# amberxie88/latent_diffusion_planning

Measured on AMD Instinct MI355X. Metric: latent plans/sec (horizon=9, 100 DDIM steps), higher is better.
Workload: dtype f32; 1 GPU; configs[1]: rm_lift planner ConditionalUnet1D (D=25, T=8, down_dims [256,512,1024]), 100-step DDIM, batch 256 synthetic latents per GPU, random-init weights, Philox noise, hipGraph-captured loop; plans_per_gpu=256, denoise_steps=100, sampler=ddim, graph=True, parallelism=dp1, ranks_seen_by_backend=1, backend=none, range_fallback=0, fp16_plane_launches=0

## Files before the change

### latent_diffusion_planning_amd/csrc/engine.hip

```cpp
#include "engine.hpp"
#include "sconv.hpp"
#include "t2pack.hpp"
#include "t4pack.hpp"
#include "version.h"

#include <algorithm>
#include <cmath>
#include <cstring>

namespace ldp {

void betas_squaredcos(int n, std::vector<float>& betas, std::vector<float>& alphas,
                             std::vector<float>& acp) {
  auto abar = [](double t) {
    const double c = std::cos((t + 0.008) / 1.008 * M_PI / 2.0);
    return c * c;
  };
  betas.resize(n);
  alphas.resize(n);
  acp.resize(n);
  float run = 1.0f;
  for (int i = 0; i < n; ++i) {
    const double b = std::min(1.0 - abar((double)(i + 1) / n) / abar((double)i / n), 0.999);
    betas[i] = (float)b;
    alphas[i] = 1.0f - betas[i];
    run = run * alphas[i];
    acp[i] = run;
  }
}

void make_step_coefs(int n_train, int n_steps, int sampler, std::vector<StepCoef>& out) {
  std::vector<float> betas, alphas, acp;
  betas_squaredcos(n_train, betas, alphas, acp);
  out.assign(n_steps, StepCoef{});
  const int stride = n_train / n_steps;
  for (int i = 0; i < n_steps; ++i) {
// ... 187 lines not shown
  const HostTensor& t = it->second;
  if (t.shape.size() != shape.size() || !std::equal(shape.begin(), shape.end(), t.shape.begin())) {
    std::string got, want;
    for (auto s : t.shape) got += std::to_string(s) + ",";
    for (auto s : shape) want += std::to_string(s) + ",";
    return fail(LDP_EINVAL, "weight '%s' has shape (%s) expected (%s)", path.c_str(), got.c_str(),
                want.c_str());
  }
  *out = &t;
  return LDP_OK;
}

static int upload_padded(DevBuf& dst, const float* src, int n, int n_p, float fill, hipStream_t s) {
  std::vector<float> tmp(n_p, fill);
  std::copy(src, src + n, tmp.begin());
  LDP_TRY(dst.alloc((size_t)n_p * 4));
  LDP_HIP(hipMemcpy(dst.p, tmp.data(), (size_t)n_p * 4, hipMemcpyHostToDevice));
  (void)s;
  return LDP_OK;
}

int make_conv(ldp_handle* h, const std::string& prefix, int nj, int cin, int cout, int cin_p,
              int cout_p, const char* gn_prefix, hipStream_t s, ConvW& out, int t_pos) {
  const HostTensor *k = nullptr, *b = nullptr;
  LDP_TRY(get_weight(h, prefix + "/kernel", &k, {nj, cin, cout}));
  LDP_TRY(get_weight(h, prefix + "/bias", &b, {cout}));
  out.t2s = nj == 5 && t2_shared(MODE_K5, t_pos, 0);
  out.t4s = nj == 5 && t4_shared(MODE_K5, t_pos, 0);
  std::vector<float> packed = out.t2s ? pack_conv_t2(k->data.data(), nullptr, cin, cout, cin_p, cout_p)
                            : out.t4s ? pack_conv_t4(k->data.data(), nullptr, cin, cout, cin_p, cout_p)
                                      : pack_conv(k->data.data(), nj, cin, cout, cin_p, cout_p);
  LDP_TRY(out.w.alloc(packed.size() * 4));
  LDP_HIP(hipMemcpy(out.w.p, packed.data(), packed.size() * 4, hipMemcpyHostToDevice));
  LDP_TRY(upload_padded(out.bias, b->data.data(), cout, cout_p, 0.f, s));
  out.nj = nj; out.cin = cin; out.cout = cout; out.cin_p = cin_p; out.cout_p = cout_p;
  out.has_gn = gn_prefix != nullptr;
  out.wsplit.release(); out.wsplit16.release(); out.wsplit16h.release(); out.wsplith.release();
  out.f16_refused = false;
  if (gn_prefix) {
    const HostTensor *gs = nullptr, *gb = nullptr;
    LDP_TRY(get_weight(h, std::string(gn_prefix) + "/scale", &gs, {cout}));
    LDP_TRY(get_weight(h, std::string(gn_prefix) + "/bias", &gb, {cout}));
    LDP_TRY(upload_padded(out.gn_scale, gs->data.data(), cout, cout_p, 1.f, s));
    LDP_TRY(upload_padded(out.gn_bias, gb->data.data(), cout, cout_p, 0.f, s));
  }
  return LDP_OK;
}

static int add_res_proj(ldp_handle* h, const std::string& conv_prefix, const std::string& prefix, int cin,
                        int cout, int cin_p, ConvW& c) {
  const HostTensor *k = nullptr, *b = nullptr, *kc = nullptr;
  LDP_TRY(get_weight(h, prefix + "/kernel", &k, {1, cin, cout}));
  LDP_TRY(get_weight(h, prefix + "/bias", &b, {cout}));
  LDP_TRY(get_weight(h, conv_prefix + "/kernel", &kc, {c.nj, cin, cout}));
  c.wsplit.release(); c.wsplit16.release(); c.wsplit16h.release(); c.wsplith.release();
  c.f16_refused = false;
  std::vector<float> packed;
  if (c.t2s) {
    packed = pack_conv_t2(kc->data.data(), k->data.data(), cin, cout, cin_p, c.cout_p);
  } else if (c.t4s) {
    packed = pack_conv_t4(kc->data.data(), k->data.data(), cin, cout, cin_p, c.cout_p);
  } else {
    std::vector<float> both(kc->data);
    both.insert(both.end(), k->data.begin(), k->data.end());
    packed = pack_conv(both.data(), c.nj + 1, cin, cout, cin_p, c.cout_p);
  }
  LDP_TRY(c.w.alloc(packed.size() * 4));
  LDP_HIP(hipMemcpy(c.w.p, packed.data(), packed.size() * 4, hipMemcpyHostToDevice));
  LDP_TRY(c.bres.alloc((size_t)cout * 4));
  LDP_HIP(hipMemcpy(c.bres.p, b->data.data(), (size_t)cout * 4, hipMemcpyHostToDevice));
  c.has_res = true;
  return LDP_OK;
}

static int round_up(int v, int m) { return (v + m - 1) / m * m; }

static int pick_plan(int mode, int to, int cout, int cin_total, int ca, bool res_out, ConvPlan& p,
                     int* cs_io = nullptr, int mb_want = 1, bool up_full_depth = false) {
  const int gw = cout >= 256 ? cout / 8 : 32;
  if (cs_io && *cs_io == 4) {
    const int qb = gw / 4;
    int ks4 = 0, cpi4 = 0;
    if (mode == MODE_K5) {
      if (to == 2 && qb == 32) { ks4 = 4; cpi4 = 2; }
      else if (to == 4 && qb == 16) { ks4 = 8; cpi4 = 1; }
      else if (to == 8 && qb == 16) { ks4 = 8; cpi4 = 1; }
      else if (to == 4 && qb == 32) { ks4 = 4; cpi4 = res_out ? 1 : 2; }
    }
    const int chunk4 = 16 * ks4 * cpi4;
// ... 63 lines not shown
    else if (to == 4 && bn == 128) { ks = 1; cpi = 2; }
    else if (to == 4 && bn == 32) { if (cin_total % 128 == 0) { ks = 4; cpi = 2; } else { ks = 2; cpi = 1; } }
    else if (to == 2 && bn == 32) { ks = 4; cpi = 1; }
  }
  if (ks == 0)
    return fail(LDP_EINVAL, "no MFMA conv instantiation for mode=%d T_out=%d C_out=%d (group width %d)",
                mode, to, cout, bn);
  p = ConvPlan{mode, to, nwn, ks, cpi, res_out ? 1 : 0};
  if (mb_want == 2 && mode == MODE_K5 &&
      ((to == 4 && !res_out && (bn == 64 || bn == 32)) || (to == 2 && (bn == 128 || bn == 64))))
    p.mb = 2;
  if (cin_total % p.chunk() != 0 || ca % p.chunk() != 0)
    return fail(LDP_EINVAL, "input channels (%d, first part %d) not a multiple of the %d-channel chunk "
                "(mode=%d T_out=%d C_out=%d)", cin_total, ca, p.chunk(), mode, to, cout);
  return LDP_OK;
}

static int launch_conv(ldp_handle* h, const ConvPlan& p, const ConvArgs& a_in, hipStream_t s) {
  const int dbg = h->opt.dbg, repeat = h->opt.repeat;
  ConvArgs a = a_in;
  a.dbg = dbg;
  if (h->opt.timeline_ptr && h->last_conv_launches < 64)
    a.tl = reinterpret_cast<unsigned long long*>(h->opt.timeline_ptr) + (size_t)h->last_conv_launches * 131072;
  if (!(a.flags & EP_STEP))
    for (int i = 1; i < repeat; ++i) (void)tconv_launch(p, a, s);
  const int r = tconv_launch(p, a, s);
  h->plan_log[plan_key(p)]++;
  h->last_conv_launches++;
  h->last_total_launches++;
  if (p.mb == 2 && p.to == 4 && (p.split == 2 || p.split == 3)) h->stat_mb2_launches++;
  if (p.split >= 3) h->stat_f16_launches++;
  if (t2_shared(p.mode, p.to, p.split)) h->stat_t2_shared_launches++;
  if (t4_shared(p.mode, p.to, p.split)) h->stat_t4_shared_launches++;
  if (r == -100)
    return fail(LDP_EINVAL, "conv instantiation missing: mode=%d TO=%d NWN=%d KS=%d CPI=%d res=%d",
                p.mode, p.to, p.nwn, p.ks, p.cpi, p.res_out);
  if (r != 0) return fail(LDP_EHIP, "conv launch failed: %s", hipGetErrorString((hipError_t)r));
  return LDP_OK;
}

static int block_positions(const PlannerState& P, size_t i) {
  const int nd = 2 * P.L;
  const int lvl = (int)i < nd ? (int)i / 2 : (int)i < nd + 2 ? P.L - 1 : P.L - 1 - ((int)i - nd - 2) / 2;
  return P.T >> lvl;
}

int planner_finalize(ldp_handle* h, hipStream_t s) {
  const ldp_config& c = h->cfg;
  PlannerState& P = h->pl;
  P = PlannerState{};
  P.D = c.obs_dim; P.DP = round_up(c.obs_dim, 32); P.G = c.global_cond_dim; P.T = c.pred_horizon;
  P.L = c.n_levels; P.E = c.step_embed_dim; P.n_train = c.planner_train_steps;
  P.C0P = P.DP <= 32 ? 128 : round_up(P.DP, 64);
  if (c.kernel_size != 5 || c.n_groups != 8)
    return fail(LDP_EINVAL, "only kernel_size=5 / n_groups=8 kernels are built (got %d / %d)",
                c.kernel_size, c.n_groups);
  if (P.L < 2 || P.L > LDP_MAX_LEVELS) return fail(LDP_EINVAL, "n_levels must be 2..%d", LDP_MAX_LEVELS);
  if (P.T % (1 << (P.L - 1)) != 0)
    return fail(LDP_EINVAL, "pred_horizon=%d is not a multiple of %d: the reference U-Net's skip "
                "connections cannot be concatenated (SURVEY.md fact 5)", P.T, 1 << (P.L - 1));
  P.dims.assign(c.down_dims, c.down_dims + P.L);
  for (int l = 0; l < P.L; ++l)
    if (P.dims[l] < 256 || P.dims[l] % 128 != 0)
      return fail(LDP_EINVAL, "down_dims[%d] = %d: every level must be >= 256 and a multiple of 128 "
                  "(8 GroupNorm groups of whole 16-column MFMA blocks)", l, P.dims[l]);
  const std::string root = "planner/";
// ... 383 lines not shown
    } else if (tile == 17) {
      p = ConvPlan{mode, to, p.bn() / 16, p.bn() == 32 ? 2 : 1, 2, 0};
      p.mb = 1; p.split = 1;
      a.w = w.wsplit16.f();
      if (h->f16_planner() && w.wsplit16h.p) { p.split = 3; a.w = w.wsplit16h.f(); }
      if (p.split == 3 && h->opt.planner_split_8w && ((B + 15) / 16) * 8 <= h->n_cu && ca % (32 * 2 * p.ks) == 0 &&
          ((mode == MODE_DOWN && ((to == 2 && p.nwn == 4) || (to == 4 && p.nwn == 2))) || (mode == MODE_UP && ((to == 4 && p.nwn == 4) || (to == 8 && p.nwn == 2)))))
        p.ks *= 2;
    } else if (tile == 16) {
      const int ks16 = p.bn() == 32 ? 2 : 1;
      const int cpi16 = 2;
      p = ConvPlan{MODE_K5, to, p.bn() / 16, ks16, cpi16, res_out ? 1 : 0};
      p.mb = 1; p.split = 1;
      a.w = w.wsplit16.f();
      if (h->opt.planner_split_mb2 && cs == 1 && to == 4 && p.bn() == 128 && ((B + 31) / 32) * 8 >= h->n_cu) {
        p = ConvPlan{MODE_K5, to, p.bn() / 16, 1, 2, res_out ? 1 : 0};
        p.mb = 2; p.split = 2;
      }
      if (h->f16_planner() && w.wsplit16h.p && res_out && to == 4 && p.bn() == 64 && p.cpi == 2 && p.ks == 1 && (ca + cb) % 64 == 0 && ca % 64 == 0) p.ks = 2;
      if (h->f16_planner() && w.wsplit16h.p && p.cpi == 2 && ((p.ks == 1 && (p.bn() == 128 || p.bn() == 64)) || (p.ks == 2 && (p.bn() == 32 || (p.bn() == 64 && res_out && to == 4)))) &&
          (to == 4 || to == 8 || (to == 16 && p.bn() == 32)) && !(to == 8 && p.bn() == 128)) {
        if (p.mb == 2 && res_out) p.mb = 1;
        p.split = 3;
        a.w = w.wsplit16h.f();
        if (h->opt.planner_split_8w && p.mb == 1 && p.nwn * p.ks == 4 && ((B + 15) / 16) * 8 <= h->n_cu && (ca + cb) % (32 * 2 * p.ks) == 0 && ca % (32 * 2 * p.ks) == 0 &&
            ((to == 8 && p.nwn == 2 && !res_out) || (to == 4 && p.nwn == 2) || (to == 4 && p.nwn == 4 && !res_out)))
          p.ks *= 2;
      }
    }
    if (p.split == 0 && mode == MODE_K5 && w.t2s != t2_shared(mode, to, 0))
      return fail(LDP_EINVAL, "k = 5 conv packed %s the shared-product form launched at %d positions", w.t2s ? "for" : "without", to);
    if (p.split == 0 && mode == MODE_K5 && w.t4s != t4_shared(mode, to, 0))
      return fail(LDP_EINVAL, "k = 5 conv packed %s the nine-product form launched at %d positions", w.t4s ? "for" : "without", to);
    a.bres = w.bres.f(); a.res_out = res_out;
    a.gn_scale = w.gn_scale.f(); a.gn_bias = w.gn_bias.f();
    if (film) {
      a.film_t = P.film_t.f() + film->film_off;
      a.film_g = P.film_g.f() + film->film_off;
      a.film_stride = P.F;
    }
    a.k_dev = k_dev; a.k = k;
    a.res_in = res_in; a.out = out;
    a.B = B; a.cout = w.cout_p; a.flags = flags; a.rows_valid = B * to;
    {
      const double wbytes = 4.0 * w.nj * (ca + cb) * w.cout_p, abytes = 4.0 * B * mode_ti(mode, to) * (ca + cb);
      const int thr = h->opt.by_sample;
      if (thr > 0 && a.kw <= 1 && (B + 15) / 16 <= 32768 && wbytes < (double)thr * abytes) a.by_sample = 1;
      else if (h->opt.place2d && p.split && a.kw <= 1) a.by_sample = 2;
    }
    if (!tap) return launch_conv(h, p, a, s);
    LDP_TRY(launch_conv(h, p, a, s));
    return tapped(p, a, tile, mode, to, w, xa, ca_stored, xb, cb, film);
  }

  int block(const ResBlock& b, int t, const float* xa, int ca, const float* xb, int cb, float* tmp,
            float* rbuf, float* out) {
    LDP_TRY(conv(b.c1, MODE_K5, t, xa, ca, xb, cb, tmp, EP_GN | EP_FILM, &b, nullptr,
                 b.proj ? rbuf : nullptr));
    const float* res = b.proj ? rbuf : xa;
    LDP_TRY(conv(b.c2, MODE_K5, t, tmp, b.cout, nullptr, 0, out, EP_GN | EP_RESIN, nullptr, res, nullptr));
    return LDP_OK;
  }
};
}

int planner_forward_launch(ldp_handle* h, int B, const int* k_dev, int k, bool step,
// ... 881 lines not shown
    if (v != 2) for (const auto& kv : h->plan_log) text[plan_text(kv.first)] = kv.second;
    for (const auto& kv : text) fprintf(stderr, "PLAN %s launches=%lld\n", kv.first.c_str(), (long long)kv.second);
    return LDP_OK;
  }
  else if (n == "inject_fault") { if (v && h->fault_host) h->fault_host[v == 2 ? 1 : 0] = 1u; return LDP_OK; }
  else return fail(LDP_EKEY, "unknown option '%s'", name);
  drop_graphs(h);
  return LDP_OK;
}

int ldp_get_option(ldp_handle* h, const char* name, int64_t* value) {
  if (!h || !name || !value) return fail(LDP_EINVAL, "bad argument");
  const std::string n(name);
  const Options& o = h->opt;
  if (n == "no_csplit") *value = o.no_csplit;
  else if (n == "no_mb2") *value = o.no_mb2;
  else if (n == "no_kw") *value = o.no_kw;
  else if (n == "kw_min_it") *value = o.kw_min_it;
  else if (n == "kw_bmax") *value = o.kw_bmax;
  else if (n == "no_fin_rows") *value = o.no_fin_rows;
  else if (n == "no_batch_split") *value = o.no_batch_split;
  else if (n == "up_full_depth") *value = o.up_full_depth;
  else if (n == "planner_split") *value = o.planner_split;
  else if (n == "planner_split_updown") *value = o.planner_split_updown;
  else if (n == "planner_split_cs2") *value = o.planner_split_cs2;
  else if (n == "planner_split_c256") *value = o.planner_split_c256;
  else if (n == "planner_split_mb2") *value = o.planner_split_mb2;
  else if (n == "planner_split_t2res") *value = o.planner_split_t2res;
  else if (n == "planner_split_t16") *value = o.planner_split_t16;
  else if (n == "planner_split_f16") *value = o.planner_split_f16;
  else if (n == "stat_f16_launches") *value = h->stat_f16_launches;
  else if (n == "stat_t2_shared_launches") *value = h->stat_t2_shared_launches;
  else if (n == "stat_t4_shared_launches") *value = h->stat_t4_shared_launches;
  else if (n == "stat_mb2_launches") *value = h->stat_mb2_launches;
  else if (n.rfind("stat_train_gemm_", 0) == 0) {
    static const char* const forms[3] = {"nn", "nt", "tn"};
    static const char* const tiles[5] = {"32", "32_ki2", "64", "64_ki2", "128"};
    const std::string rest = n.substr(16);
    int idx = rest == "fused" ? LDP_STAT_GEMM_FUSED : rest == "reduce" ? LDP_STAT_GEMM_REDUCE : -1;
    for (int f = 0; f < 3 && idx < 0; ++f)
      for (int t = 0; t < 5; ++t)
        if (rest == std::string(forms[f]) + "_" + tiles[t]) idx = f * 5 + t;
    if (idx < 0) return fail(LDP_EKEY, "unknown option '%s'", name);
    *value = h->stat_train_gemm[idx];
  }
  else if (n.rfind("stat_idm_", 0) == 0) {
    const std::string rest = n.substr(9);
    int idx = rest == "unfused" ? LDP_STAT_IDM_UNFUSED : rest == "f16_hs2" ? LDP_STAT_IDM_F16_HS2 : rest == "f16_hs4" ? LDP_STAT_IDM_F16_HS4 : -1;
    for (int hs = 1; hs <= 8 && idx < 0; hs *= 2)
      for (int ring = 0; ring <= (hs >= 4 ? 1 : 0); ++ring)
        for (int nt = 0; nt < 2; ++nt)
          if (rest == "f32_hs" + std::to_string(hs) + (ring ? "_ring" : "") + (nt ? "_nt" : "")) idx = stat_idm_f32(hs, ring != 0, nt != 0);
    if (idx < 0) return fail(LDP_EKEY, "unknown option '%s'", name);
    *value = h->stat_idm[idx];
  }
  else if (n == "vae_no_conv_stats") *value = o.vae_no_conv_stats;
  else if (n == "vae_no_conv_in_stats") *value = o.vae_no_conv_in_stats;
  else if (n == "vae_split") *value = o.vae_split;
  else if (n == "vae_split_f16") *value = o.vae_split_f16;
  else if (n == "vae_split_gn_only") *value = o.vae_split_gn_only;
  else if (n == "vae_split_s2") *value = o.vae_split_s2;
  else if (n == "timeline_ptr") *value = o.timeline_ptr;
  else if (n == "idm_unfused") *value = o.idm_unfused;
  else if (n == "idm_rt_major") *value = o.idm_rt_major;
  else if (n == "idm_noring") *value = o.idm_noring;
  else if (n == "idm_stream") *value = o.idm_stream;
// ... 37 lines not shown
                   int64_t n, void* stream) {
  if (!out_dev || n <= 0) return fail(LDP_EINVAL, "bad argument");
  return philox_raw_launch(seed, elem0, step, stream_id, out_dev, n, (hipStream_t)stream);
}

int ldp_philox_normal(uint64_t seed, uint64_t elem0, uint32_t step, uint32_t stream_id, float* out_dev,
                      int64_t n, void* stream) {
  if (!out_dev || n <= 0) return fail(LDP_EINVAL, "bad argument");
  return philox_normal_launch(seed, elem0, step, stream_id, out_dev, n, (hipStream_t)stream);
}

int ldp_launch_count(ldp_handle* h, int32_t which, int64_t* launches) {
  if (!h || !launches) return fail(LDP_EINVAL, "bad argument");
  *launches = which == 0 ? h->last_conv_launches : h->last_total_launches;
  return LDP_OK;
}

static int prim_conv(int mode, const float* x, const float* kernel_host, const float* bias_host,
                     const float* gs, const float* gb, const float* film, float* y, int B, int t_in,
                     int cin, int cout, void* stream) {
  if (!x || !kernel_host || !bias_host || !y || B <= 0) return fail(LDP_EINVAL, "bad argument");
  hipStream_t s = (hipStream_t)stream;
  const int nj = mode_taps(mode);
  const int to = mode == MODE_DOWN ? t_in / 2 : mode == MODE_UP ? t_in * 2 : t_in;
  if (cout % 128 != 0) return fail(LDP_EINVAL, "Cout must be a multiple of 128 (8 groups x 16)");
  ConvPlan p;
  int cin_pp = round_up(cin, 32);
  for (int pad = 64; pick_plan(mode, to, cout, cin_pp, cin_pp, false, p) != LDP_OK; pad *= 2) {
    if (pad > 256) return LDP_EINVAL;
    cin_pp = round_up(cin, pad);
  }
  std::vector<float> packed = t2_shared(mode, to, 0) ? pack_conv_t2(kernel_host, nullptr, cin, cout, cin_pp, cout)
                            : t4_shared(mode, to, 0) ? pack_conv_t4(kernel_host, nullptr, cin, cout, cin_pp, cout)
                                                     : pack_conv(kernel_host, nj, cin, cout, cin_pp, cout);
  DevBuf dw, db, dgs, dgb, dx, dfg, dft;
  LDP_TRY(upload(dw, packed.data(), packed.size() * 4, s));
  LDP_TRY(upload(db, bias_host, (size_t)cout * 4, s));
  ConvArgs a{};
  if (gs) {
    LDP_TRY(upload(dgs, gs, (size_t)cout * 4, s));
    LDP_TRY(upload(dgb, gb, (size_t)cout * 4, s));
    a.flags |= EP_GN;
  }
  const float* xin = x;
  if (cin_pp != cin) {
    LDP_TRY(dx.alloc((size_t)B * t_in * cin_pp * 4));
    LDP_TRY(pad_rows_launch(x, dx.f(), (int64_t)B * t_in, cin, cin_pp, s));
    xin = dx.f();
  }
  if (film) {
    LDP_TRY(dft.alloc((size_t)2 * cout * 4));
    LDP_HIP(hipMemsetAsync(dft.p, 0, (size_t)2 * cout * 4, s));
    a.film_t = dft.f(); a.film_g = film; a.film_stride = 2 * cout; a.flags |= EP_FILM;
  }
  a.xa = xin; a.ca = cin_pp; a.w = dw.f(); a.bias = db.f();
  a.gn_scale = dgs.f(); a.gn_bias = dgb.f();
  a.out = y; a.B = B; a.cout = cout; a.k = 0; a.rows_valid = B * to;
  const int r = tconv_launch(p, a, s);
  if (r != 0) return fail(r == -100 ? LDP_EINVAL : LDP_EHIP, "primitive conv launch failed (%d)", r);
  LDP_HIP(hipStreamSynchronize(s));
  return LDP_OK;
}

int ldp_conv1d_gn_mish_film_f32(const float* x, const float* kernel_host, const float* bias_host,
                                const float* gn_scale_host, const float* gn_bias_host,
                                const float* film, float* y, int32_t B, int32_t T, int32_t Cin,
// ... 19 lines not shown
```

### latent_diffusion_planning_amd/csrc/engine.hpp

```cpp
#pragma once
#include <functional>
#include <map>
#include <memory>
#include <string>
#include <vector>

#include "common.hpp"
#include "tconv.hpp"

namespace ldp {

struct HostTensor {
  std::vector<int64_t> shape;
  std::vector<float> data;
  int64_t numel() const {
    int64_t n = 1;
    for (auto s : shape) n *= s;
    return n;
  }
};

struct ConvW {
  DevBuf w, bias, gn_scale, gn_bias, bres;
  DevBuf wsplit;
  DevBuf wsplith;
  DevBuf wsplit16h;
  DevBuf wsplit16;
  bool f16_refused = false;
  int nj = 0, cin = 0, cout = 0, cin_p = 0, cout_p = 0;
  bool has_gn = false, has_res = false;
  bool t2s = false;
  bool t4s = false;
};

struct ResBlock {
  ConvW c1, c2;
  bool proj = false;
  int cin = 0, cout = 0;
  int film_off = 0;
  std::string prefix;
};

struct PlannerState {
  bool ready = false;
  int D = 0, DP = 0, G = 0, T = 0, L = 0, E = 0, n_train = 0;
  int C0P = 128;
  std::vector<int> dims;
  std::vector<ResBlock> blocks;
  std::vector<ConvW> down, up;
  ConvW fin_block, fin_conv;
  int F = 0;
  DevBuf film_t;
  DevBuf wfilm_g;
  int ws_B = 0;
  DevBuf state, cond, film_g, bufA, bufB, bufC, bufR, noise, xchg, kw_slab;
  DevBuf solver_eps, solver_x0;
  DevBuf ctarget, cmask;
  DevBuf gtarget, gwg, ganchor;
  DevBuf gcol;
  size_t xchg_stride = 0;
  uint64_t calls = 0;
  std::vector<DevBuf> skip;
};

struct IdmState {
// ... 107 lines not shown
  std::map<std::string, ldp::HostTensor> weights;
  ldp::PlannerState pl;
  ldp::IdmState idm;
  ldp::DevBuf seed;
  uint64_t epoch_planner = 0, epoch_idm = 0;
  uint64_t* ctl_planner() const { return seed.as<uint64_t>(); }
  uint64_t* ctl_idm() const { return seed.as<uint64_t>() + 4; }
  volatile unsigned int* fault_host = nullptr;
  unsigned int* fault_dev = nullptr;
  int fault_pending = 0;
  int64_t faults_seen = 0;
  bool safe_mode = false;
  bool range_fallback = false;
  int64_t range_faults_seen = 0;
  unsigned int* range_dev() const { return fault_dev ? fault_dev + 1 : nullptr; }
  bool f16_planner() const { return opt.planner_split_f16 != 0 && !range_fallback; }
  bool f16_vae() const { return opt.vae_split_f16 != 0 && !range_fallback; }
  ldp::Options opt;
  std::map<int, ldp::SolverTable> solver_tabs;
  ldp::DevBuf plan_out, act_out, obs_last;
  ldp::DevBuf cand_cond;
  ldp::DevBuf slot_buf;
  hipStream_t cap_stream = nullptr;
  int n_cu = 256;
  std::map<ldp::GraphKey, ldp::GraphEntry> graphs;
  std::vector<ldp::GraphEntry> retired_execs;
  uint64_t graph_clock = 0;
  int graph_cap = 32;
  int64_t graphs_captured = 0, graphs_evicted = 0;
  int64_t last_conv_launches = 0, last_total_launches = 0;
  int64_t stat_f16_launches = 0;
  int64_t stat_t2_shared_launches = 0;
  int64_t stat_t4_shared_launches = 0;
  std::map<uint64_t, int64_t> plan_log;
  int64_t stat_mb2_launches = 0;
  int64_t stat_train_gemm[17] = {};
  int64_t stat_idm[19] = {};
  void* vae = nullptr;
  void* train = nullptr;
  void* resnet = nullptr;
};

namespace ldp {
std::map<std::string, int64_t> tconv_plan_log();
uint64_t plan_key(const ConvPlan& p);
std::string plan_text(uint64_t key);
void make_step_coefs(int n_train, int n_steps, int sampler, std::vector<StepCoef>& out);
void sinusoid_table(int n, int dim, bool cos_first, std::vector<float>& out);

std::vector<float> pack_conv(const float* w, int nj, int cin, int cout, int cin_p, int cout_p);

bool fits_f16_planes(const float* w, size_t n);
std::vector<uint16_t> pack_conv_split16h(const float* w, int nj, int cin, int cout);
int get_weight(ldp_handle* h, const std::string& path, const HostTensor** out,
               std::initializer_list<int64_t> shape);
int make_conv(ldp_handle* h, const std::string& prefix, int nj, int cin, int cout, int cin_p,
              int cout_p, const char* gn_prefix, hipStream_t s, ConvW& out, int t_pos = 0);

void drop_graphs(ldp_handle* h);
void reap_retired_graphs(ldp_handle* h);
inline int bucket_rows(int B, bool explicit_noise) { return explicit_noise ? B : (B + 15) / 16 * 16; }
struct LoopSpec { int n_steps = 0, sampler = 0; bool explicit_noise = false; int begin = 0, end = -1; int constrain = 0; int guide = 0; };
inline bool stepped_loop(const LoopSpec& L) { return L.guide != 0 || L.sampler == LDP_SAMPLER_DPMPP; }
constexpr int LDP_GUIDE_ON = 1, LDP_GUIDE_ANCHOR = 2;
int check_step_range(int begin, int end, int n_steps, const char* what);
struct WarmSpec;
// ... 72 lines not shown
```

### latent_diffusion_planning_amd/csrc/tconv.hpp

```cpp
#pragma once
#include <hip/hip_runtime.h>
#include <stdint.h>
#include <type_traits>

#pragma clang fp contract(off)

#ifndef LDP_W_NT
#define LDP_W_NT 0
#endif
#ifndef LDP_SPLIT_NPROD
#define LDP_SPLIT_NPROD 6
#endif
#ifndef LDP_S16_LF
#define LDP_S16_LF 100
#endif
#ifndef LDP_F16_MINW
#define LDP_F16_MINW 2
#endif
#ifndef LDP_RANGE_GUARD
#define LDP_RANGE_GUARD 1
#endif
#ifndef LDP_KERNARG_TOUCH
#define LDP_KERNARG_TOUCH 1
#endif
// ... 113 lines not shown
  const int ti_n = mode_ti(mode, to_n);
  for (int to = 0; to < to_n; ++to) {
    const int ti = tap_src(mode, to, j);
    if (ti >= 0 && ti < ti_n) return true;
  }
  return false;
}
__host__ __device__ constexpr int valid_pairs(int mode, int to_n) {
  const int ti_n = mode_ti(mode, to_n);
  int n = 0;
  for (int to = 0; to < to_n; ++to)
    for (int j = 0; j < mode_taps(mode); ++j) {
      const int ti = tap_src(mode, to, j);
      if (ti >= 0 && ti < ti_n) ++n;
    }
  return n;
}

#ifndef LDP_T2_DIRECT
#define LDP_T2_DIRECT 0
#endif
__host__ __device__ constexpr bool t2_shared(int mode, int to_n, int split) {
  return !LDP_T2_DIRECT && mode == MODE_K5 && to_n == 2 && split == 0;
}
constexpr int T2_SLOTS = 3;

#ifndef LDP_T4_DIRECT
#define LDP_T4_DIRECT 0
#endif
__host__ __device__ constexpr bool t4_shared(int mode, int to_n, int split) {
  return !LDP_T4_DIRECT && mode == MODE_K5 && to_n == 4 && split == 0;
}
constexpr int T4_SLOTS = 9;
__host__ __device__ constexpr int conv_products(int mode, int to_n, int split) {
  return t2_shared(mode, to_n, split) ? T2_SLOTS : t4_shared(mode, to_n, split) ? T4_SLOTS : valid_pairs(mode, to_n);
}

__device__ __forceinline__ int swz(int row, int slot) { return slot ^ ((4 - (row >> 2)) & 3); }

#ifndef LDP_EPILOGUE_IEEE
#define LDP_EPILOGUE_IEEE 0
#endif
__device__ __forceinline__ float mish_f(float x) {
#if LDP_EPILOGUE_IEEE
  const float e = expf(fminf(x, 20.0f));
  const float n = e * (e + 2.0f);
  return x * (n / (n + 2.0f));
#else
  const float e = __builtin_amdgcn_exp2f(fminf(x, 20.0f) * 1.4426950408889634f);
  const float n = e * (e + 2.0f);
  return x * (n * __builtin_amdgcn_rcpf(n + 2.0f));
#endif
}

template <int CTRL, int ROW_MASK>
__device__ __forceinline__ float dpp_add(float v) {
  return v + __int_as_float(__builtin_amdgcn_update_dpp(0, __float_as_int(v), CTRL, ROW_MASK, 0xF, false));
}
__device__ __forceinline__ float wave_sum(float v) {
  v = dpp_add<0xB1, 0xF>(v);
  v = dpp_add<0x4E, 0xF>(v);
  v = dpp_add<0x114, 0xF>(v);
  v = dpp_add<0x118, 0xF>(v);
  v = dpp_add<0x142, 0xA>(v);
  v = dpp_add<0x143, 0xC>(v);
  return __int_as_float(__builtin_amdgcn_readlane(__float_as_int(v), 63));
// ... 173 lines not shown
  if (sb * (16 * MB) >= a.B) return;
  const int cbk = grp * cs + half;
  const int b0 = sb * (16 * MB);
  const int r = lane & 15, kq = lane >> 4;
  const int nblk_total = S32 ? a.cout >> 5 : a.cout >> 4;
  const int nblk = cbk * C::NWC + wn;
  const int cin = a.ca + a.cb;
  int nit_all = LDP_ABL(8) ? 0 : (mode_2d(MODE) ? 3 * cin : cin) / C::CH_IT;
  if constexpr (MODE == MODE_K5 && RES_OUT && SPLIT == 0 && !KWS) {
    if (a.ca_real > 0 && !LDP_ABL(8)) nit_all = (a.ca_real + C::CH_IT - 1) / C::CH_IT;
  }
  const int it0 = kpart * (nit_all / kw);
  const int nit = it0 + nit_all / kw;
  if LDP_ABL(64) return;
  LDP_TL(0);

  constexpr bool T2S = t2_shared(MODE, TO, SPLIT);
  f32x4 acc[MB][TO];
  f32x4 racc[MB][RES_OUT ? TO : 1];
  f32x4 sacc[T2S ? MB : 1];
  constexpr bool T2S2 = T2S && KS == 1 && CPI % 2 == 0;
  f32x4 sacc_b[T2S2 ? MB : 1], acc_b[T2S2 ? MB : 1][2];
#pragma unroll
  for (int m = 0; m < (T2S ? MB : 1); ++m) sacc[m] = f32x4{0.f, 0.f, 0.f, 0.f};
#pragma unroll
  for (int m = 0; m < (T2S2 ? MB : 1); ++m) sacc_b[m] = acc_b[m][0] = acc_b[m][1] = f32x4{0.f, 0.f, 0.f, 0.f};
  constexpr bool T4S = t4_shared(MODE, TO, SPLIT);
  constexpr bool T4F = T4S && KS == 1 && !RES_OUT;
  constexpr bool T4P = T4S && MB == 2;
  constexpr int MBE = T4P ? 1 : MB;
  constexpr int NLDE = T4P ? C::NLD / 2 : C::NLD;
  static_assert(!T4P || C::NLD % 2 == 0, "two-pass tiles: whole staging loads per row block");
  static_assert(!(T4P && (T4F || RES_OUT)), "two-pass tiles: K slices, no projection");
  f32x4 tacc[T4S && !T4F ? MBE : 1][T4S && !T4F ? T4_SLOTS : 1];
#pragma unroll
  for (int m = 0; m < (T4S && !T4F ? MBE : 1); ++m)
#pragma unroll
    for (int t = 0; t < (T4S && !T4F ? T4_SLOTS : 1); ++t) tacc[m][t] = f32x4{0.f, 0.f, 0.f, 0.f};
  f32x4 acc_lo[C::F16 ? MB : 1][C::F16 ? TO : 1], racc_lo[C::F16 ? MB : 1][C::F16 && RES_OUT ? TO : 1];
#pragma unroll
  for (int m = 0; m < (C::F16 ? MB : 1); ++m) {
#pragma unroll
    for (int t = 0; t < (C::F16 ? TO : 1); ++t) acc_lo[m][t] = f32x4{0.f, 0.f, 0.f, 0.f};
#pragma unroll
    for (int t = 0; t < (C::F16 && RES_OUT ? TO : 1); ++t) racc_lo[m][t] = f32x4{0.f, 0.f, 0.f, 0.f};
  }
#pragma unroll
  for (int m = 0; m < MB; ++m) {
#pragma unroll
    for (int t = 0; t < TO; ++t) acc[m][t] = f32x4{0.f, 0.f, 0.f, 0.f};
#pragma unroll
    for (int t = 0; t < (RES_OUT ? TO : 1); ++t) racc[m][t] = f32x4{0.f, 0.f, 0.f, 0.f};
  }

  int st_goff[C::NLD];
  int st_loff[C::NLD];
  int st_cc[C::NLD];
  int st_mask[mode_2d(MODE) ? C::NLD : 1];
#pragma unroll
  for (int i = 0; i < C::NLD; ++i) {
    const int idx = tid + i * NT;
    const int q = idx & 3;
    const int cc = (idx >> 2) % NC;
    const int rr = (idx / (4 * NC)) & 15;
    const int tm = idx / (64 * NC);
    const int tt = tm % TI, mb = tm / TI;
// ... 41 lines not shown
    for (int i = SI0; i < SI1; ++i) {
      const bool ok = (cbase + st_cc[i]) < creal;
      xst[i] = *reinterpret_cast<const f32x4*>(base + (size_t)st_goff[i] * stride + (ok ? cbase + st_cc[i] : 0));
    }
  };
  auto stage_store = [&](auto pass_tag, float* buf) {
    constexpr int SI0 = T4P ? decltype(pass_tag)::value * (C::NLD / 2) : 0, SI1 = T4P ? SI0 + C::NLD / 2 : C::NLD;
    if constexpr (C::F16) {
#pragma unroll
      for (int i = 0; i < C::NLD; ++i) {
        uint2 ph, pl;
        split4h(xst[i], ph, pl);
        *reinterpret_cast<uint2*>(buf + st_loff[i]) = ph;
        *reinterpret_cast<uint2*>(buf + st_loff[i] + 256) = pl;
      }
      return;
    }
    if constexpr (SPLIT) {
#pragma unroll
      for (int i = 0; i < C::NLD; ++i) {
        uint2 ph, pm, pl;
        split4(xst[i], ph, pm, pl);
        *reinterpret_cast<uint2*>(buf + st_loff[i]) = ph;
        *reinterpret_cast<uint2*>(buf + st_loff[i] + 256) = pm;
        *reinterpret_cast<uint2*>(buf + st_loff[i] + 512) = pl;
      }
      return;
    }
#pragma unroll
    for (int i = SI0; i < SI1; ++i) *reinterpret_cast<f32x4*>(buf + st_loff[i]) = xst[i];
  };

  constexpr bool SKIPZ = MODE == MODE_K5 && RES_OUT && SPLIT == 0 && TO >= 8 && KS > 1;
  constexpr int NJR = T2S ? T2_SLOTS : T4S ? T4_SLOTS : NJ;
  constexpr int NJW = NJR + (RES_OUT ? 1 : 0);
  constexpr int NJB = T4S ? T4_SLOTS : NJ;
  constexpr int NSTEP = S16 ? CPI / 2 : 1;
  constexpr int WCH = S16 ? 1 : CPI;
  constexpr int RN = RES_OUT ? WCH : 1;
  constexpr int WPL = SPLIT ? C::NPL : 1;
  f32x4 wb0[NJB][WCH * WPL], wb1[NJB][WCH * WPL];
  f32x4 rb0[RN * WPL], rb1[RN * WPL];
  auto wload = [&](int it, f32x4 (&b)[NJB][WCH * WPL], f32x4 (&rb)[RN * WPL]) {
#pragma unroll
    for (int ci = 0; ci < WCH; ++ci) {
      const int gc = S16 ? (it / NSTEP) * (NC / 2) + ks * NSTEP + (it % NSTEP) : it * NC + ks * CPI + ci;
#pragma unroll
      for (int j = 0; j < NJB; ++j) {
        if constexpr (SPLIT) {
          if (tap_used(MODE, TO, j)) {
#pragma unroll
            for (int pl = 0; pl < WPL; ++pl) {
              const size_t off = ((((size_t)gc * NJW + j) * nblk_total + nblk) * WPL + pl) * 256 + lane * 4;
              b[j][ci * WPL + pl] = *reinterpret_cast<const f32x4*>(a.w + off);
            }
          }
        } else
        if (T4S || tap_used(MODE, TO, j)) {
          const size_t off = (((size_t)gc * NJW + (T2S ? j - 1 : j)) * nblk_total + nblk) * 256 + lane * 4;
          b[j][ci] = (LDP_W_NT && KWS) ? __builtin_nontemporal_load(reinterpret_cast<const f32x4*>(a.w + off))
                                       : *reinterpret_cast<const f32x4*>(a.w + off);
        }
      }
      if constexpr (RES_OUT && SPLIT) {
#pragma unroll
        for (int pl = 0; pl < WPL; ++pl) {
          const size_t off = ((((size_t)gc * NJW + NJ) * nblk_total + nblk) * WPL + pl) * 256 + lane * 4;
          rb[ci * WPL + pl] = *reinterpret_cast<const f32x4*>(a.w + off);
        }
      } else
      if (RES_OUT) {
        const size_t off = (((size_t)gc * NJW + NJR) * nblk_total + nblk) * 256 + lane * 4;
        rb[ci] = (LDP_W_NT && KWS) ? __builtin_nontemporal_load(reinterpret_cast<const f32x4*>(a.w + off))
                                   : *reinterpret_cast<const f32x4*>(a.w + off);
      }
    }
  };

  f32x16 acc32[S32 ? TO : 1], racc32[S32 && RES_OUT ? TO : 1];
  f32x16 acc32_lo[S32 && C::F16 ? TO : 1], racc32_lo[S32 && C::F16 && RES_OUT ? TO : 1];
  if constexpr (S32 && C::F16) {
#pragma unroll
    for (int t = 0; t < TO; ++t)
#pragma unroll
      for (int i = 0; i < 16; ++i) acc32_lo[t][i] = 0.f;
#pragma unroll
    for (int t = 0; t < (RES_OUT ? TO : 1); ++t)
#pragma unroll
      for (int i = 0; i < 16; ++i) racc32_lo[t][i] = 0.f;
  }
  if constexpr (S32) {
#pragma unroll
    for (int t = 0; t < TO; ++t)
#pragma unroll
      for (int i = 0; i < 16; ++i) acc32[t][i] = 0.f;
#pragma unroll
    for (int t = 0; t < (RES_OUT ? TO : 1); ++t)
#pragma unroll
      for (int i = 0; i < 16; ++i) racc32[t][i] = 0.f;
  }
  auto iteration = [&](auto pass_tag, auto last_tag, int it, f32x4 (&bc)[NJB][WCH * WPL], f32x4 (&rc)[RN * WPL], f32x4 (&bl)[NJB][WCH * WPL],
                       f32x4 (&rl)[RN * WPL]) {
    constexpr bool LAST = decltype(last_tag)::value;
    constexpr int PASS = decltype(pass_tag)::value;
    float* xcur = smem + (it & 1) * C::XT;
    float* xnext = smem + ((it + 1) & 1) * C::XT;
    const int itn = LDP_ABL(256) ? it0 : (LAST || (it + 1) < nit) ? it + 1 : it;
    if (!LAST) {
      if (!(SPLIT && LDP_ABL(2048))) stage_load(pass_tag, itn);
      if (!S16 && !(SPLIT && LDP_ABL(1024))) wload(itn, bl, rl);
    }
    if constexpr (S16) {
      constexpr int NPAIR = valid_pairs(MODE, TO) + (RES_OUT ? TO : 0);
      constexpr int NUSED = (tap_used(MODE, TO, 0) ? 1 : 0) + (NJ > 1 && tap_used(MODE, TO, 1) ? 1 : 0) + (NJ > 2 && tap_used(MODE, TO, 2) ? 1 : 0) +
                            (NJ > 3 && tap_used(MODE, TO, 3) ? 1 : 0) + (NJ > 4 && tap_used(MODE, TO, 4) ? 1 : 0);
      constexpr int NPL = C::NPL;
      constexpr int NWL = (NUSED + (RES_OUT ? 1 : 0)) * NPL;
      constexpr int NMFMA = (C::F16 ? 3 : LDP_SPLIT_NPROD) * NPAIR * MB;
      constexpr int NREAD = MB * TI * NPL;
      constexpr int AHEAD = MB * (TI > 2 ? 2 : TI) * NPL;
      auto step = [&](auto pc_tag, f32x4 (&wc)[NJB][WCH * WPL], f32x4 (&rcur)[RN * WPL], f32x4 (&wn)[NJB][WCH * WPL], f32x4 (&rnext)[RN * WPL]) {
        constexpr int pc = decltype(pc_tag)::value;
        constexpr bool PREF = pc + 1 < NSTEP || !LAST;
        if (PREF && !LDP_ABL(1024)) wload(pc + 1 < NSTEP ? it * NSTEP + pc + 1 : itn * NSTEP, wn, rnext);
        f32x4 asp[MB][TI][NPL];
#pragma unroll
        for (int ti = 0; ti < TI; ++ti) {
#pragma unroll
          for (int m = 0; m < MB; ++m)
#pragma unroll
            for (int pl = 0; pl < NPL; ++pl)
              asp[m][ti][pl] = *reinterpret_cast<const f32x4*>(xcur + (((((m * TI + ti) * (NC / 2) + ks * NSTEP + pc) * NPL + pl) * 64 + lane) * 4));
        }
        if constexpr (C::F16) {
          constexpr int FA[3] = {1, 0, 0}, FB[3] = {0, 1, 0};
#pragma unroll
          for (int ti = 0; ti < TI; ++ti) {
#pragma unroll
            for (int pi = 0; pi < 3; ++pi) {
#pragma unroll
              for (int j = 0; j <= NJ; ++j) {
                if (j == NJ && !RES_OUT) continue;
                const int to = j == NJ ? (ti < TO ? ti : -1) : tap_dst(MODE, TO, ti, j < NJ ? j : 0);
// ... 189 lines not shown
          af[mm][3] = x2 + x3; af[mm][4] = x3; af[mm][5] = x2;
          af[mm][6] = x0 + x1; af[mm][7] = x1; af[mm][8] = x0;
        }
#pragma unroll
        for (int s = 0; s < 4; ++s) {
#pragma unroll
          for (int k = 0; k < T4_SLOTS; ++k) {
#pragma unroll
            for (int m = 0; m < MBE; ++m) {
              f32x4& d = T4F ? tit[T4F ? m : 0][T4F ? k : 0] : tacc[T4F ? 0 : m][T4F ? 0 : k];
              d = __builtin_amdgcn_mfma_f32_16x16x4f32(af[m][k][s], bc[k][ci][s], d, 0, 0, 0);
            }
          }
          if (RES_OUT) {
#pragma unroll
            for (int to = 0; to < TO; ++to)
#pragma unroll
              for (int m = 0; m < MB; ++m)
                racc[m][to] = __builtin_amdgcn_mfma_f32_16x16x4f32(areg[m][to][ci][s], rc[ci][s], racc[m][to], 0, 0, 0);
          }
        }
      }
      if constexpr (T4F) {
#pragma unroll
        for (int m = 0; m < MB; ++m) {
          const f32x4 se0 = tit[m][0] + tit[m][1], se1 = tit[m][0] + tit[m][2];
          acc[m][0] = acc[m][0] + ((se0 + tit[m][3]) + tit[m][4]);
          acc[m][1] = acc[m][1] + ((se1 + tit[m][3]) + tit[m][5]);
          acc[m][2] = acc[m][2] + ((se0 + tit[m][6]) + tit[m][7]);
          acc[m][3] = acc[m][3] + ((se1 + tit[m][6]) + tit[m][8]);
        }
      }
    } else
    if (!dead_slice) {
#pragma unroll
    for (int ci = 0; ci < CPI; ++ci) {
#pragma unroll
      for (int s = 0; s < 4; ++s) {
#pragma unroll
        for (int j = 0; j < NJ; ++j) {
#pragma unroll
          for (int to = 0; to < TO; ++to) {
            const int ti = tap_src(MODE, to, j);
            if (ti >= 0 && ti < TI) {
#pragma unroll
              for (int m = 0; m < MB; ++m)
                acc[m][to] = __builtin_amdgcn_mfma_f32_16x16x4f32(areg[m][ti][ci][s], bc[j][ci][s],
                                                                  acc[m][to], 0, 0, 0);
            }
          }
        }
        if (RES_OUT) {
#pragma unroll
          for (int to = 0; to < TO; ++to)
#pragma unroll
            for (int m = 0; m < MB; ++m)
              racc[m][to] = __builtin_amdgcn_mfma_f32_16x16x4f32(areg[m][to][ci][s], rc[ci][s],
                                                                 racc[m][to], 0, 0, 0);
        }
      }
    }
    }
    if (LAST) {
#pragma unroll
      for (int i = 0; i < MBE * TI * CPI; ++i) __builtin_amdgcn_sched_group_barrier(0x100, 1, 0);
    } else {
      constexpr int NUSED = (tap_used(MODE, TO, 0) ? 1 : 0) + (NJ > 1 && tap_used(MODE, TO, 1) ? 1 : 0) +
                            (NJ > 2 && tap_used(MODE, TO, 2) ? 1 : 0) + (NJ > 3 && tap_used(MODE, TO, 3) ? 1 : 0) +
                            (NJ > 4 && tap_used(MODE, TO, 4) ? 1 : 0);
      constexpr int NLOADS = NLDE + ((T4S ? T4_SLOTS : NUSED) + (RES_OUT ? 1 : 0)) * CPI;
      constexpr int NMFMA = MBE * CPI * 4 * (conv_products(MODE, TO, SPLIT) + (RES_OUT ? TO : 0));
      constexpr int MPL = NMFMA / NLOADS > 0 ? NMFMA / NLOADS : 1;
#pragma unroll
      for (int i = 0; i < MBE * TI * CPI; ++i) __builtin_amdgcn_sched_group_barrier(0x100, 1, 0);
#pragma unroll
      for (int i = 0; i < NLOADS; ++i) {
        __builtin_amdgcn_sched_group_barrier(0x020, 1, 0);
        __builtin_amdgcn_sched_group_barrier(0x008, MPL, 0);
      }
      if (NMFMA - NLOADS * MPL > 0) __builtin_amdgcn_sched_group_barrier(0x008, NMFMA - NLOADS * MPL, 0);
      __builtin_amdgcn_sched_group_barrier(0x200, NLDE, 0);
    }
    if (!LAST) stage_store(pass_tag, xnext);
    __syncthreads();
  };

#define LDP_TCONV_PASS(pass_tag) \
  stage_load(pass_tag, it0); \
  wload(S16 ? it0 * NSTEP : it0, wb0, rb0); \
  stage_store(pass_tag, smem + (it0 & 1) * C::XT); \
  __syncthreads(); \
  LDP_TL(1); \
  if (mode_2d(MODE) && !S16) { \
    for (int it = it0; it < nit; it += 2) { \
      iteration(pass_tag, std::false_type{}, it, wb0, rb0, wb1, rb1); \
// ... 516 lines not shown
            (t_landed & 0xffffffffffffull) | (drain << 48);
    }
#endif
    if (C::STATS) {
      if (a.stats_part) {
        float* sp = smem + C::TILE_FLOATS;
        sp[wave * 64 + lane] = gs1;
        sp[(C::NW + wave) * 64 + lane] = gs2;
        __syncthreads();
        if (tid < 128) {
          const int which = tid >> 6, c = tid & 63;
          float t = 0.f;
#pragma unroll
          for (int w = 0; w < C::NW; ++w) t += sp[(which * C::NW + w) * 64 + c];
          a.stats_part[((size_t)sb * a.cout + cbk * BN + c) * 2 + which] = t;
        }
      }
    }
  }
}

__host__ __device__ constexpr bool tconv_kw_ok(int mode, int to, int nwn, int mb) {
  return (mode == MODE_K5 || mode == MODE_DOWN || mode == MODE_UP) && mb == 1 && to * 16 * nwn <= 512;
}

struct ConvPlan {
  int mode, to, nwn, ks, cpi, res_out;
  int mb = 1;
  int kws = 0;
  int split = 0;
  int bn() const { return 16 * nwn; }
  int chunk() const { return 16 * ks * cpi; }
};
int tconv_launch(const ConvPlan& p, const ConvArgs& a, hipStream_t stream);
int tconv_init_all();
int tconv_init_k5();
int tconv_init_k5r();
int tconv_init_misc();
int tconv_init_2d();
int tconv_launch_2d(const ConvPlan& p, const ConvArgs& a, hipStream_t stream);
int tconv_launch_k5(const ConvPlan& p, const ConvArgs& a, hipStream_t stream);
int tconv_launch_k5r(const ConvPlan& p, const ConvArgs& a, hipStream_t stream);
int tconv_launch_misc(const ConvPlan& p, const ConvArgs& a, hipStream_t stream);
int tconv_launch_split(const ConvPlan& p, const ConvArgs& a, hipStream_t stream);
int tconv_init_split();

}
```

Baseline: 5844 plans/s.

## Add a shared-product form for k=5 convs at eight positions

Adds a 13-slot weight packing and a kernel path for k=5 convolutions over 8 output positions without a residual projection. Each half of the tile reuses the 4-position Winograd-like nine-product combination, and two extra slots cover taps that cross the halves. This cuts MFMA work from the direct tap-by-position products to 24 products per sub-chunk. In exchange it stores an extra packed weight copy, adds input pre-additions, hand-schedules the weight prefetch across the compute groups, and changes how floating-point sums are ordered.

```diff
diff --git a/latent_diffusion_planning_amd/csrc/engine.hip b/latent_diffusion_planning_amd/csrc/engine.hip
--- a/latent_diffusion_planning_amd/csrc/engine.hip
+++ b/latent_diffusion_planning_amd/csrc/engine.hip
@@ -2,6 +2,7 @@
 #include "sconv.hpp"
 #include "t2pack.hpp"
 #include "t4pack.hpp"
+#include "t8pack.hpp"
 #include "version.h"
 
 #include <algorithm>
@@ -255,6 +256,13 @@
                                       : pack_conv(k->data.data(), nj, cin, cout, cin_p, cout_p);
   LDP_TRY(out.w.alloc(packed.size() * 4));
   LDP_HIP(hipMemcpy(out.w.p, packed.data(), packed.size() * 4, hipMemcpyHostToDevice));
+  out.w8.release();
+  out.t8s = nj == 5 && t8_shared(MODE_K5, t_pos, 0);
+  if (out.t8s) {
+    const std::vector<float> p8 = pack_conv_t8(k->data.data(), cin, cout, cin_p, cout_p);
+    LDP_TRY(out.w8.alloc(p8.size() * 4));
+    LDP_HIP(hipMemcpy(out.w8.p, p8.data(), p8.size() * 4, hipMemcpyHostToDevice));
+  }
   LDP_TRY(upload_padded(out.bias, b->data.data(), cout, cout_p, 0.f, s));
   out.nj = nj; out.cin = cin; out.cout = cout; out.cin_p = cin_p; out.cout_p = cout_p;
   out.has_gn = gn_prefix != nullptr;
@@ -278,6 +286,7 @@
   LDP_TRY(get_weight(h, conv_prefix + "/kernel", &kc, {c.nj, cin, cout}));
   c.wsplit.release(); c.wsplit16.release(); c.wsplit16h.release(); c.wsplith.release();
   c.f16_refused = false;
+  c.w8.release(); c.t8s = false;
   std::vector<float> packed;
   if (c.t2s) {
     packed = pack_conv_t2(kc->data.data(), k->data.data(), cin, cout, cin_p, c.cout_p);
@@ -407,6 +416,7 @@
   if (p.split >= 3) h->stat_f16_launches++;
   if (t2_shared(p.mode, p.to, p.split)) h->stat_t2_shared_launches++;
   if (t4_shared(p.mode, p.to, p.split)) h->stat_t4_shared_launches++;
+  if (t8_plan(p)) h->stat_t8_shared_launches++;
   if (r == -100)
     return fail(LDP_EINVAL, "conv instantiation missing: mode=%d TO=%d NWN=%d KS=%d CPI=%d res=%d",
                 p.mode, p.to, p.nwn, p.ks, p.cpi, p.res_out);
@@ -856,6 +866,10 @@
       return fail(LDP_EINVAL, "k = 5 conv packed %s the shared-product form launched at %d positions", w.t2s ? "for" : "without", to);
     if (p.split == 0 && mode == MODE_K5 && w.t4s != t4_shared(mode, to, 0))
       return fail(LDP_EINVAL, "k = 5 conv packed %s the nine-product form launched at %d positions", w.t4s ? "for" : "without", to);
+    if (t8_plan(p)) {
+      if (!w.t8s || !w.w8.p) return fail(LDP_EINVAL, "k = 5 conv without the 24-product packing launched on a tile that takes the form (%d positions)", to);
+      a.w = w.w8.f();
+    }
     a.bres = w.bres.f(); a.res_out = res_out;
     a.gn_scale = w.gn_scale.f(); a.gn_bias = w.gn_bias.f();
     if (film) {
@@ -1803,6 +1817,7 @@
   else if (n == "stat_f16_launches") *value = h->stat_f16_launches;
   else if (n == "stat_t2_shared_launches") *value = h->stat_t2_shared_launches;
   else if (n == "stat_t4_shared_launches") *value = h->stat_t4_shared_launches;
+  else if (n == "stat_t8_shared_launches") *value = h->stat_t8_shared_launches;
   else if (n == "stat_mb2_launches") *value = h->stat_mb2_launches;
   else if (n.rfind("stat_train_gemm_", 0) == 0) {
     static const char* const forms[3] = {"nn", "nt", "tn"};
@@ -1906,6 +1921,7 @@
   }
   std::vector<float> packed = t2_shared(mode, to, 0) ? pack_conv_t2(kernel_host, nullptr, cin, cout, cin_pp, cout)
                             : t4_shared(mode, to, 0) ? pack_conv_t4(kernel_host, nullptr, cin, cout, cin_pp, cout)
+                            : t8_plan(p)             ? pack_conv_t8(kernel_host, cin, cout, cin_pp, cout)
                                                      : pack_conv(kernel_host, nj, cin, cout, cin_pp, cout);
   DevBuf dw, db, dgs, dgb, dx, dfg, dft;
   LDP_TRY(upload(dw, packed.data(), packed.size() * 4, s));
diff --git a/latent_diffusion_planning_amd/csrc/engine.hpp b/latent_diffusion_planning_amd/csrc/engine.hpp
--- a/latent_diffusion_planning_amd/csrc/engine.hpp
+++ b/latent_diffusion_planning_amd/csrc/engine.hpp
@@ -31,6 +31,8 @@
   bool has_gn = false, has_res = false;
   bool t2s = false;
   bool t4s = false;
+  DevBuf w8;
+  bool t8s = false;
 };
 
 struct ResBlock {
@@ -204,6 +206,7 @@
   int64_t stat_f16_launches = 0;
   int64_t stat_t2_shared_launches = 0;
   int64_t stat_t4_shared_launches = 0;
+  int64_t stat_t8_shared_launches = 0;
   std::map<uint64_t, int64_t> plan_log;
   int64_t stat_mb2_launches = 0;
   int64_t stat_train_gemm[17] = {};
diff --git a/latent_diffusion_planning_amd/csrc/t8pack.hpp b/latent_diffusion_planning_amd/csrc/t8pack.hpp
--- /dev/null
+++ b/latent_diffusion_planning_amd/csrc/t8pack.hpp
@@ -0,0 +1,39 @@
+#pragma once
+#include <cstddef>
+#include <vector>
+
+#include "t4pack.hpp"
+
+namespace ldp {
+
+constexpr int T8_PACK_SLOTS = 13;
+
+inline void t8_combine(const float w[5], float out[T8_PACK_SLOTS]) {
+  t4_combine(w, out);
+  out[9] = w[0];
+  out[10] = w[1];
+  out[11] = w[3];
+  out[12] = w[4];
+}
+
+inline std::vector<float> pack_conv_t8(const float* w, int cin, int cout, int cin_p, int cout_p) {
+  const int nchunk = cin_p / 16, nblk = cout_p / 16, ns = T8_PACK_SLOTS;
+  std::vector<float> p((size_t)nchunk * ns * nblk * 256, 0.0f);
+  for (int gc = 0; gc < nchunk; ++gc)
+    for (int nb = 0; nb < nblk; ++nb)
+      for (int lane = 0; lane < 64; ++lane) {
+        const int kq = lane >> 4, n = lane & 15;
+        const int co = nb * 16 + n;
+        for (int s = 0; s < 4; ++s) {
+          const int ci = gc * 16 + 4 * kq + s;
+          if (ci >= cin || co >= cout) continue;
+          float taps[5], v[T8_PACK_SLOTS];
+          for (int j = 0; j < 5; ++j) taps[j] = w[((size_t)j * cin + ci) * cout + co];
+          t8_combine(taps, v);
+          for (int sl = 0; sl < ns; ++sl) p[(((size_t)gc * ns + sl) * nblk + nb) * 256 + lane * 4 + s] = v[sl];
+        }
+      }
+  return p;
+}
+
+}
diff --git a/latent_diffusion_planning_amd/csrc/tconv.hpp b/latent_diffusion_planning_amd/csrc/tconv.hpp
--- a/latent_diffusion_planning_amd/csrc/tconv.hpp
+++ b/latent_diffusion_planning_amd/csrc/tconv.hpp
@@ -169,6 +169,18 @@
   return !LDP_T4_DIRECT && mode == MODE_K5 && to_n == 4 && split == 0;
 }
 constexpr int T4_SLOTS = 9;
+
+#ifndef LDP_T8_DIRECT
+#define LDP_T8_DIRECT 0
+#endif
+__host__ __device__ constexpr bool t8_shared(int mode, int to_n, int split) {
+  return !LDP_T8_DIRECT && mode == MODE_K5 && to_n == 8 && split == 0;
+}
+constexpr int T8_SLOTS = 13;
+__device__ constexpr int T8_ORDER[T8_SLOTS] = {11, 0, 1, 2, 12, 3, 4, 5, 6, 7, 8, 9, 10};
+__host__ __device__ constexpr bool t8_tile(int mode, int to_n, int split, int nwn, int ks, int cpi, bool res_out, int mb, bool kws) {
+  return t8_shared(mode, to_n, split) && !res_out && mb == 1 && cpi == 1;
+}
 __host__ __device__ constexpr int conv_products(int mode, int to_n, int split) {
   return t2_shared(mode, to_n, split) ? T2_SLOTS : t4_shared(mode, to_n, split) ? T4_SLOTS : valid_pairs(mode, to_n);
 }
@@ -408,6 +420,7 @@
   constexpr int NLDE = T4P ? C::NLD / 2 : C::NLD;
   static_assert(!T4P || C::NLD % 2 == 0, "two-pass tiles: whole staging loads per row block");
   static_assert(!(T4P && (T4F || RES_OUT)), "two-pass tiles: K slices, no projection");
+  constexpr bool T8S = t8_tile(MODE, TO, SPLIT, NWN, KS, CPI, RES_OUT, MB, KWS);
   f32x4 tacc[T4S && !T4F ? MBE : 1][T4S && !T4F ? T4_SLOTS : 1];
 #pragma unroll
   for (int m = 0; m < (T4S && !T4F ? MBE : 1); ++m)
@@ -515,9 +528,9 @@
   };
 
   constexpr bool SKIPZ = MODE == MODE_K5 && RES_OUT && SPLIT == 0 && TO >= 8 && KS > 1;
-  constexpr int NJR = T2S ? T2_SLOTS : T4S ? T4_SLOTS : NJ;
+  constexpr int NJR = T2S ? T2_SLOTS : T4S ? T4_SLOTS : T8S ? T8_SLOTS : NJ;
   constexpr int NJW = NJR + (RES_OUT ? 1 : 0);
-  constexpr int NJB = T4S ? T4_SLOTS : NJ;
+  constexpr int NJB = T4S ? T4_SLOTS : T8S ? T8_SLOTS : NJ;
   constexpr int NSTEP = S16 ? CPI / 2 : 1;
   constexpr int WCH = S16 ? 1 : CPI;
   constexpr int RN = RES_OUT ? WCH : 1;
@@ -529,7 +542,8 @@
     for (int ci = 0; ci < WCH; ++ci) {
       const int gc = S16 ? (it / NSTEP) * (NC / 2) + ks * NSTEP + (it % NSTEP) : it * NC + ks * CPI + ci;
 #pragma unroll
-      for (int j = 0; j < NJB; ++j) {
+      for (int jj = 0; jj < NJB; ++jj) {
+        const int j = T8S ? T8_ORDER[jj % T8_SLOTS] : jj;
         if constexpr (SPLIT) {
           if (tap_used(MODE, TO, j)) {
 #pragma unroll
@@ -539,7 +553,7 @@
             }
           }
         } else
-        if (T4S || tap_used(MODE, TO, j)) {
+        if (T4S || T8S || tap_used(MODE, TO, j)) {
           const size_t off = (((size_t)gc * NJW + (T2S ? j - 1 : j)) * nblk_total + nblk) * 256 + lane * 4;
           b[j][ci] = (LDP_W_NT && KWS) ? __builtin_nontemporal_load(reinterpret_cast<const f32x4*>(a.w + off))
                                        : *reinterpret_cast<const f32x4*>(a.w + off);
@@ -591,7 +605,7 @@
     const int itn = LDP_ABL(256) ? it0 : (LAST || (it + 1) < nit) ? it + 1 : it;
     if (!LAST) {
       if (!(SPLIT && LDP_ABL(2048))) stage_load(pass_tag, itn);
-      if (!S16 && !(SPLIT && LDP_ABL(1024))) wload(itn, bl, rl);
+      if (!S16 && !T8S && !(SPLIT && LDP_ABL(1024))) wload(itn, bl, rl);
     }
     if constexpr (S16) {
       constexpr int NPAIR = valid_pairs(MODE, TO) + (RES_OUT ? TO : 0);
@@ -847,6 +861,66 @@
         }
       }
     } else
+    if constexpr (T8S) {
+      static_assert(MB == 1 && CPI == 1 && !RES_OUT, "24-product form: one row block, one sub-chunk per iteration, no projection");
+      const int gcn = itn * NC + ks * CPI;
+      auto wl = [&](int j) {
+        bl[j][0] = *reinterpret_cast<const f32x4*>(a.w + (((size_t)gcn * NJW + j) * nblk_total + nblk) * 256 + lane * 4);
+      };
+      constexpr int RC[2][3] = {{11, 12, 12}, {9, 10, 9}};
+      __builtin_amdgcn_sched_barrier(0);
+#pragma unroll
+      for (int hf = 0; hf < 2; ++hf) {
+        f32x4 tit[T4_SLOTS + 2];
+#pragma unroll
+        for (int k = 0; k < T4_SLOTS + 2; ++k) tit[k] = f32x4{0.f, 0.f, 0.f, 0.f};
+        const f32x4 x0 = areg[0][4 * hf][0], x1 = areg[0][4 * hf + 1][0], x2 = areg[0][4 * hf + 2][0], x3 = areg[0][4 * hf + 3][0];
+        const f32x4 cx0 = areg[0][hf == 0 ? 4 : 2][0], cx1 = areg[0][hf == 0 ? 5 : 3][0];
+#pragma unroll
+        for (int g = 0; g < 3; ++g) {
+          f32x4 af[3];
+          if (g == 0) {
+            const f32x4 u0 = x0 + x2, u1 = x1 + x3;
+            af[0] = u0 + u1; af[1] = u1; af[2] = u0;
+          } else if (g == 1) {
+            af[0] = x2 + x3; af[1] = x3; af[2] = x2;
+          } else {
+            af[0] = x0 + x1; af[1] = x1; af[2] = x0;
+          }
+          const f32x4 cx = g == 0 ? cx0 : g == 1 ? cx1 : hf == 0 ? cx0 : cx1;
+          const int ct = g == 2 ? 9 : 10;
+#pragma unroll
+          for (int s = 0; s < 4; ++s) {
+#pragma unroll
+            for (int k = 0; k < 3; ++k)
+              tit[3 * g + k] = __builtin_amdgcn_mfma_f32_16x16x4f32(af[k][s], bc[3 * g + k][0][s], tit[3 * g + k], 0, 0, 0);
+            tit[ct] = __builtin_amdgcn_mfma_f32_16x16x4f32(cx[s], bc[RC[hf][g]][0][s], tit[ct], 0, 0, 0);
+          }
+          __builtin_amdgcn_sched_barrier(0);
+          if (!LAST && hf == 1) {
+            if (g == 0) { wl(11); wl(0); wl(1); wl(2); wl(12); }
+            if (g == 1) { wl(3); wl(4); wl(5); }
+            if (g == 2) { wl(6); wl(7); wl(8); wl(9); wl(10); }
+            __builtin_amdgcn_sched_barrier(0);
+          }
+        }
+        const f32x4 se0 = tit[0] + tit[1], se1 = tit[0] + tit[2];
+        const f32x4 y0 = (se0 + tit[3]) + tit[4], y1 = (se1 + tit[3]) + tit[5];
+        const f32x4 y2 = (se0 + tit[6]) + tit[7], y3 = (se1 + tit[6]) + tit[8];
+        if (hf == 0) {
+          acc[0][0] = acc[0][0] + y0;
+          acc[0][1] = acc[0][1] + y1;
+          acc[0][2] = acc[0][2] + (y2 + tit[9]);
+          acc[0][3] = acc[0][3] + (y3 + tit[10]);
+        } else {
+          acc[0][4] = acc[0][4] + (y0 + tit[10]);
+          acc[0][5] = acc[0][5] + (y1 + tit[9]);
+          acc[0][6] = acc[0][6] + y2;
+          acc[0][7] = acc[0][7] + y3;
+        }
+        __builtin_amdgcn_sched_barrier(0);
+      }
+    } else
     if (!dead_slice) {
 #pragma unroll
     for (int ci = 0; ci < CPI; ++ci) {
@@ -876,6 +950,8 @@
       }
     }
     }
+    if constexpr (T8S) {
+    } else
     if (LAST) {
 #pragma unroll
       for (int i = 0; i < MBE * TI * CPI; ++i) __builtin_amdgcn_sched_group_barrier(0x100, 1, 0);
@@ -1458,6 +1534,7 @@
   int bn() const { return 16 * nwn; }
   int chunk() const { return 16 * ks * cpi; }
 };
+inline bool t8_plan(const ConvPlan& p) { return t8_tile(p.mode, p.to, p.split, p.nwn, p.ks, p.cpi, p.res_out != 0, p.mb, p.kws != 0); }
 int tconv_launch(const ConvPlan& p, const ConvArgs& a, hipStream_t stream);
 int tconv_init_all();
 int tconv_init_k5();
```

New measurement: 5800 plans/s. About the same (-0.7%).
